# joejep/FOCNeRF

Hardware: AMD Instinct MI355X
Metric: train_samples_per_sec (higher is better)
Workload: dtype f16

## Files before the change

focnerf_amd/_lib.py:

```python
import ctypes
import os

import torch

_HERE = os.path.dirname(os.path.abspath(__file__))
LIB_PATH = os.environ.get("FOCNERF_LIB_PATH") or os.path.join(_HERE, "libfocnerf_hip.so")

c_u8p = ctypes.c_void_p
c_vp = ctypes.c_void_p
u32 = ctypes.c_uint32
u64 = ctypes.c_uint64
f32 = ctypes.c_float
i32 = ctypes.c_int

FOC_F32 = 0
FOC_F16 = 1



class FocOccTrainNode(ctypes.Structure):
    _fields_ = [
        ("struct_bytes", u32),
        ("n_rays", u32), ("max_steps", u32), ("cascade", u32), ("grid_size", u32), ("cap", u32), ("pad_align", u32),
        ("bound", f32), ("dt_gamma", f32), ("min_near", f32),
# ... 47 lines not shown
    _fields_ = [
        ("mask", c_vp), ("offsets", c_vp), ("sigma_c", c_vp), ("rgb_c", c_vp),
        ("m_occ", u32), ("density_scale", f32), ("thresh", f32), ("sigma_gain", f32),
    ]


SIGNATURES = {
    "foc_abi_version": (i32, []),
    "foc_last_error": (ctypes.c_char_p, []),
    "foc_arch": (ctypes.c_char_p, []),
    "foc_near_far_from_aabb": (i32, [c_vp, c_vp, c_vp, u32, f32, c_vp, c_vp, c_vp]),
    "foc_sph_from_ray": (i32, [c_vp, c_vp, f32, u32, c_vp, c_vp]),
    "foc_morton3D": (i32, [c_vp, u32, c_vp, c_vp]),
    "foc_morton3D_invert": (i32, [c_vp, u32, c_vp, c_vp]),
    "foc_packbits": (i32, [c_vp, u32, f32, c_vp, c_vp]),
    "foc_march_rays_train": (i32, [c_vp, c_vp, c_vp, f32, f32, u32, u32, u32, u32, u32, c_vp, c_vp,
                                   c_vp, c_vp, c_vp, c_vp, c_vp, c_vp, c_vp, c_vp]),
    "foc_march_rays_train_field": (i32, [c_vp, c_vp, c_vp, f32, f32, u32, u32, u32, u32, u32, c_vp, c_vp,
                                         c_vp, c_vp, c_vp, c_vp, c_vp, c_vp, c_vp, u32, c_vp, f32, c_vp]),
    "foc_set_option": (i32, [ctypes.c_char_p, i32]),
    "foc_get_option": (i32, [ctypes.c_char_p, c_vp]),
    "foc_guard_pick_device": (i32, [i32, i32, i32, i32]),
    "foc_grid_forward_index_path": (i32, [u32, u32, u32]),
    "foc_view_tile_order": (i32, [c_vp, u32, u32, u32, c_vp, c_vp, c_vp]),
    "foc_occ_train_forward": (i32, [ctypes.POINTER(FocOccTrainNode), c_vp]),
    "foc_occ_train_backward": (i32, [ctypes.POINTER(FocOccTrainNode), c_vp]),
    "foc_occ_train_forward_pad31": (i32, [ctypes.POINTER(FocOccTrainNode), f32, c_vp]),
    "foc_occ_train_backward_pad31": (i32, [ctypes.POINTER(FocOccTrainNode), f32, c_vp]),
    "foc_occ_train_forward_obj": (i32, [ctypes.POINTER(FocOccTrainNode), ctypes.POINTER(FocOccTrainObject), c_vp]),
    "foc_occ_train_backward_obj": (i32, [ctypes.POINTER(FocOccTrainNode), ctypes.POINTER(FocOccTrainObject), c_vp]),
    "foc_occ_tail_forward_sumsq": (i32, [c_vp, c_vp, u32, c_vp, c_vp, u32, u32, f32, f32, c_vp, f32, c_vp, c_vp, c_vp, c_vp, c_vp, c_vp, c_vp, c_vp]),
    "foc_occ_tail_backward_sumsq": (i32, [c_vp, c_vp, c_vp, c_vp, u32, c_vp, c_vp, c_vp, c_vp, c_vp, u32, u32, f32, f32, c_vp, f32, c_vp, c_vp, c_vp, c_vp]),
    "foc_occ_tail_forward": (i32, [c_vp, c_vp, u32, c_vp, c_vp, u32, u32, f32, f32, c_vp, f32, c_vp, c_vp, c_vp, c_vp, c_vp, c_vp, c_vp]),
    "foc_occ_tail_backward": (i32, [c_vp, c_vp, c_vp, c_vp, u32, c_vp, c_vp, c_vp, c_vp, c_vp, u32, u32, f32, f32, c_vp, f32, c_vp, c_vp, c_vp]),
    "foc_occ_tail_forward_dist": (i32, [c_vp, c_vp, u32, c_vp, c_vp, u32, u32, f32, f32, c_vp, f32, c_vp, c_vp, c_vp, c_vp, c_vp, c_vp, c_vp, c_vp, c_vp,
                                        c_vp]),
    "foc_occ_tail_backward_dist": (i32, [c_vp, c_vp, c_vp, c_vp, u32, c_vp, c_vp, c_vp, c_vp, c_vp, u32, u32, f32, f32, c_vp, f32, c_vp, c_vp, c_vp, c_vp,
                                         c_vp, c_vp, c_vp]),
    "foc_occ_tail_forward_depth": (i32, [c_vp, c_vp, u32, c_vp, c_vp, u32, u32, f32, f32, c_vp, f32, c_vp, c_vp, c_vp, c_vp, c_vp, c_vp, c_vp, c_vp, c_vp,
                                         c_vp, c_vp]),
    "foc_occ_tail_backward_depth": (i32, [c_vp, c_vp, c_vp, c_vp, u32, c_vp, c_vp, c_vp, c_vp, c_vp, u32, u32, f32, f32, c_vp, f32, c_vp, c_vp, c_vp, c_vp,
                                          c_vp, c_vp, c_vp, c_vp, c_vp, c_vp, c_vp]),
    "foc_occ_train_forward_tail": (i32, [ctypes.POINTER(FocOccTrainNode), ctypes.POINTER(FocOccTrainObject), f32, ctypes.POINTER(FocOccTrainTail), c_vp]),
    "foc_occ_train_backward_tail": (i32, [ctypes.POINTER(FocOccTrainNode), ctypes.POINTER(FocOccTrainObject), f32, ctypes.POINTER(FocOccTrainTail), c_vp]),
    "foc_march_rays_train_scratch_bytes": (u64, [u32, u32]),
    "foc_composite_rays_train_forward": (i32, [c_vp, c_vp, c_vp, c_vp, u32, u32, f32, c_vp, c_vp, c_vp, c_vp]),
# ... 223 lines not shown
```

focnerf_amd/csrc/combine.hip:

```cpp
#include "common.h"
#include "fs_common.h"
#include <string.h>
#include <cmath>

static thread_local char g_err[512] = "";

void foc_set_error(const char *fmt, ...) {
    va_list ap;
    va_start(ap, fmt);
    vsnprintf(g_err, sizeof(g_err), fmt, ap);
    va_end(ap);
}

__global__ void __launch_bounds__(256) k_combine_select(const float *__restrict__ dens, const float *__restrict__ rgb,
                                                        float *__restrict__ max_dens, float *__restrict__ best_rgb, uint64_t n) {
    for (uint64_t i = (uint64_t)blockIdx.x * 256 + threadIdx.x; i < n; i += (uint64_t)gridDim.x * 256) {
        const float d = dens[i], m = max_dens[i];
        if (d > m) { best_rgb[i * 3] = rgb[i * 3]; best_rgb[i * 3 + 1] = rgb[i * 3 + 1]; best_rgb[i * 3 + 2] = rgb[i * 3 + 2]; }
        max_dens[i] = (d != d || m != m) ? __builtin_nanf("") : (d > m ? d : m);
    }
}

__global__ void __launch_bounds__(256) k_combine_pack(const float *__restrict__ dens, uint32_t rank, uint64_t *__restrict__ keys, uint64_t n) {
    for (uint64_t i = (uint64_t)blockIdx.x * 256 + threadIdx.x; i < n; i += (uint64_t)gridDim.x * 256) {
// ... 338 lines not shown
    bool take = false;
    if (s0 + lane < n) {
        const T a_raw = sig_new[s0 + lane];
        const float a = (float)a_raw, b = (float)sig_best[s0 + lane];
        take = (a != a) || (b == b && a >= b);
        if (take) sig_best[s0 + lane] = a_raw;
    }
    const uint64_t rows = __ballot(take);
    const uint32_t live = (uint32_t)(n - s0 < 64u ? n - s0 : 64u);
    const uint64_t base = s0 * width;
    for (uint32_t e = lane; e < live * width; e += 64u)
        if ((rows >> (e / width)) & 1ull) feat_best[base + e] = feat_new[base + e];
}

#include <stdlib.h>
#include <string.h>
#include <atomic>
#include <mutex>
struct FocOptionRow { const char *name; std::atomic<int> value; };
static FocOptionRow foc_option_table[FOC_OPT_COUNT] = {
    {"FOC_MLP_BWD_FUSED", 1}, {"FOC_FIELD_FWD_FUSED", 1}, {"FOC_GB_MERGE_MAX_RES", 480}, {"FOC_GB_FACTORED", 1}, {"FOC_GB_TAIL_SPLIT", 16}, {"FOC_GRID_FUSE_SMALL", 1},
    {"FOC_GRID_PAIRS", 1}, {"FOC_GRID_FAST", 1}, {"FOC_MARCH_SERIAL", -1}, {"FOC_MARCH_RAYS_ROW_MAX", 131072}, {"FOC_OCC_MARCH_FORM", -1},
    {"FOC_OCC_SAMPLE_MAJOR", 1}, {"FOC_OCC_FIELD_PIECE", 1 << 23}, {"FOC_DETERMINISTIC", 0},
};
static int foc_option_parse(int which, const char *text) {
    if (which == FOC_OPT_OCC_MARCH_FORM) {
        if (text[0] == 't') return 0;
        if (text[0] == 'r') return 1;
        if (text[0] == 'l') return 2;
        if (text[0] == 's') return 3;
    }
    return atoi(text);
}
static void foc_options_init() {
    static std::once_flag once;
    std::call_once(once, [] {
        for (int i = 0; i < FOC_OPT_COUNT; i++) {
            const char *e = getenv(foc_option_table[i].name);
            if (e && e[0]) foc_option_table[i].value.store(foc_option_parse(i, e), std::memory_order_relaxed);
        }
    });
}
int foc_opt(FocOpt which) { foc_options_init(); return foc_option_table[which].value.load(std::memory_order_relaxed); }

extern "C" {

// ... 223 lines not shown
```

focnerf_amd/csrc/common.h:

```cpp
#pragma once
#include <hip/hip_runtime.h>
#include <hip/hip_fp16.h>
#include <stdint.h>
#include <stdio.h>
#include <stdarg.h>
#include "../../include/focnerf.h"

#define FOC_WAVE 64

void foc_set_error(const char *fmt, ...);

enum FocOpt {
    FOC_OPT_MLP_BWD_FUSED,
    FOC_OPT_FIELD_FWD_FUSED,
    FOC_OPT_GB_MERGE_MAX_RES,
    FOC_OPT_GB_FACTORED,
    FOC_OPT_GB_TAIL_SPLIT,
    FOC_OPT_GRID_FUSE_SMALL,
    FOC_OPT_GRID_PAIRS,
    FOC_OPT_GRID_FAST,
    FOC_OPT_MARCH_SERIAL,
    FOC_OPT_MARCH_RAYS_ROW_MAX,
    FOC_OPT_OCC_MARCH_FORM,
    FOC_OPT_OCC_SAMPLE_MAJOR,
    FOC_OPT_OCC_FIELD_PIECE,
    FOC_OPT_DETERMINISTIC,
    FOC_OPT_COUNT
};
int foc_opt(FocOpt which);

#define FOC_REQUIRE(cond, code, ...)                    \
    do {                                                \
        if (!(cond)) {                                  \
            foc_set_error(__VA_ARGS__);                 \
            return (code);                              \
        }                                               \
    } while (0)

#define FOC_CHECK_LAUNCH(name)                                                     \
    do {                                                                           \
        hipError_t e_ = hipGetLastError();                                         \
        if (e_ != hipSuccess) {                                                    \
            foc_set_error("%s: launch failed: %s", name, hipGetErrorString(e_));   \
            return FOC_E_LAUNCH;                                                   \
        }                                                                          \
    } while (0)

static inline int foc_guard_pick(bool stream_is_null, int stream_device, int pointer_device, int current_device) {
    if (!stream_is_null && stream_device >= 0) return stream_device;
// ... 93 lines not shown
```

focnerf_amd/csrc/ge_common.h:

```cpp
#pragma once
#include "common.h"
#include <math.h>
#include <stdlib.h>

#define GE_MAX_LEVELS 32

struct GeLevels {
    float scale[GE_MAX_LEVELS];
    uint32_t resolution[GE_MAX_LEVELS];
    uint32_t merge_max_res;
};

__device__ __forceinline__ float ge_opaque(float v) { asm volatile("" : "+v"(v)); return v; }

template <typename T> struct GeT;
template <> struct GeT<float> {
    static __device__ __forceinline__ float ld(const float *p) { return *p; }
    static __device__ __forceinline__ void st(float *p, float v) { *p = v; }
};
template <> struct GeT<__half> {
    static __device__ __forceinline__ float ld(const __half *p) { return __half2float(*p); }
    static __device__ __forceinline__ void st(__half *p, float v) { *p = __float2half_rn(ge_opaque(v)); }
};

// ... 287 lines not shown
            pgl[gd] = pos_grid[gd] + 1;
            const uint32_t rr = ge_index(dim, gridtype, align_corners, hashmap_size, resolution, pgl);
            float vl[C], vr[C];
            GeVec<T, C>::ld(table + (uint64_t)rl * C, vl);
            GeVec<T, C>::ld(table + (uint64_t)rr * C, vr);
#pragma unroll
            for (uint32_t c = 0; c < C; c++) rg[c] = fmaf(w * (vr[c] - vl[c]), pos_deriv[gd], rg[c]);
        }
#pragma unroll
        for (uint32_t c = 0; c < C; c++) GeT<T>::st(dy + gd * C + c, rg[c]);
    }
}

__host__ __device__ __forceinline__ bool ge_level_hashed(uint32_t hashmap_size, uint32_t resolution, uint32_t &st1, uint32_t &st2) {
    const uint32_t r1 = resolution + 1u;
    uint32_t stride = 1u;
    st1 = st2 = 0u;
    if (stride <= hashmap_size) stride *= r1;
    if (stride <= hashmap_size) { st1 = stride; stride *= r1; }
    if (stride <= hashmap_size) { st2 = stride; stride *= r1; }
    return stride > hashmap_size;
}

__device__ __forceinline__ void ge_forward_hash3(const float (&x)[3], bool oob, const uint32_t *__restrict__ tw, uint32_t hashmap_size, bool hashed,
                                                 uint32_t st1, uint32_t st2, float scale, __half *__restrict__ out) {
    if (oob) { *reinterpret_cast<uint32_t *>(out) = 0u; return; }
    float pos[3];
    uint32_t pg[3];
#pragma unroll
    for (int d = 0; d < 3; d++) {
        const float p = fmaf(x[d], scale, 0.5f);
        pg[d] = (uint32_t)p;
        pos[d] = __builtin_amdgcn_fractf(p);
    }
    const char *tb = reinterpret_cast<const char *>(tw);
    uint32_t b0[4];
    uint2 wide[4];
    uint32_t nar[4] = {0u, 0u, 0u, 0u};
    bool pr[4];
    if (hashmap_size <= (1u << 22)) {
        const uint32_t x4 = pg[0] << 2;
        uint32_t yz4[4];
        if (hashed) {
            const uint32_t m = hashmap_size - 1u, m4 = m << 2;
            const uint32_t p1 = (2654435761u & m) << 2, p2 = (805459861u & m) << 2;
            const uint32_t t1 = __umul24(pg[1], p1), t2 = __umul24(pg[2], p2);
            yz4[0] = t1 ^ t2; yz4[1] = (t1 + p1) ^ t2; yz4[2] = t1 ^ (t2 + p2); yz4[3] = (t1 + p1) ^ (t2 + p2);
#pragma unroll
            for (int j = 0; j < 4; j++) b0[j] = (x4 ^ yz4[j]) & m4;
#pragma unroll
            for (int j = 0; j < 4; j++) wide[j] = *reinterpret_cast<const uint2 *>(tb + (b0[j] & ~7u));
            const bool even = (x4 & 4u) == 0u;
            if (!even) {
#pragma unroll
                for (int j = 0; j < 4; j++) nar[j] = *reinterpret_cast<const uint32_t *>(tb + (((x4 + 4u) ^ yz4[j]) & m4));
            }
#pragma unroll
            for (int j = 0; j < 4; j++) pr[j] = even;
        } else {
            const uint32_t s1 = st1 << 2, s2 = st2 << 2;
            const uint32_t t1 = __umul24(pg[1], s1), t2 = __umul24(pg[2], s2);
            yz4[0] = t1 + t2; yz4[1] = (t1 + s1) + t2; yz4[2] = t1 + (t2 + s2); yz4[3] = (t1 + s1) + (t2 + s2);
// ... 15 lines not shown
        for (int j = 0; j < 4; j++) b0[j] = ((pg[0] ^ yz[j]) & mask) << 2;
#pragma unroll
        for (int j = 0; j < 4; j++) wide[j] = *reinterpret_cast<const uint2 *>(tb + (b0[j] & ~7u));
        const bool even = (pg[0] & 1u) == 0u;
        if (!even) {
#pragma unroll
            for (int j = 0; j < 4; j++) nar[j] = *reinterpret_cast<const uint32_t *>(tb + ((((pg[0] + 1u) ^ yz[j]) & mask) << 2));
        }
#pragma unroll
        for (int j = 0; j < 4; j++) pr[j] = even;
    } else {
        const uint32_t t1 = pg[1] * st1, t2 = pg[2] * st2;
        const uint32_t yz[4] = {t1 + t2, (t1 + st1) + t2, t1 + (t2 + st2), (t1 + st1) + (t2 + st2)};
#pragma unroll
        for (int j = 0; j < 4; j++) b0[j] = (pg[0] + yz[j]) << 2;
#pragma unroll
        for (int j = 0; j < 4; j++) wide[j] = *reinterpret_cast<const uint2 *>(tb + (b0[j] & ~7u));
#pragma unroll
        for (int j = 0; j < 4; j++) {
            pr[j] = (b0[j] & 4u) == 0u;
            if (!pr[j]) nar[j] = *reinterpret_cast<const uint32_t *>(tb + (b0[j] + 4u));
        }
    }
    const float wx[2] = {1 - pos[0], pos[0]}, wy[2] = {1 - pos[1], pos[1]}, wz[2] = {1 - pos[2], pos[2]};
    float res0 = 0.0f, res1 = 0.0f;
#pragma unroll
    for (int j = 0; j < 4; j++) {
        const bool odd = (b0[j] & 4u) != 0u;
        const uint32_t v0 = odd ? wide[j].y : wide[j].x;
        const uint32_t v1 = pr[j] ? (odd ? wide[j].x : wide[j].y) : nar[j];
        const __half2 h0 = *reinterpret_cast<const __half2 *>(&v0), h1 = *reinterpret_cast<const __half2 *>(&v1);
        const float w0 = (wx[0] * wy[j & 1]) * wz[j >> 1], w1 = (wx[1] * wy[j & 1]) * wz[j >> 1];
        res0 = fmaf(w0, __low2float(h0), res0); res1 = fmaf(w0, __high2float(h0), res1);
        res0 = fmaf(w1, __low2float(h1), res0); res1 = fmaf(w1, __high2float(h1), res1);
    }
    *reinterpret_cast<__half2 *>(out) = __halves2half2(__float2half_rn(ge_opaque(res0)), __float2half_rn(ge_opaque(res1)));
}

__host__ __device__ __forceinline__ bool ge_hash3_admits(uint32_t hashmap_size, bool hashed) {
    return (!hashed || (hashmap_size & (hashmap_size - 1u)) == 0u) && hashmap_size <= (1u << 30);
}

template <typename T, typename DIM, uint32_t C>
__device__ __forceinline__ void ge_forward_level(DIM dim, const float (&x)[DIM::MAX], bool oob, const T *__restrict__ grid, uint32_t off0, uint32_t hashmap_size,
                                                 float scale, uint32_t resolution, T *__restrict__ out, T *__restrict__ dy, uint32_t gridtype,
                                                 bool align_corners, uint32_t interp, uint32_t pairs) {
    if constexpr (sizeof(T) == 2 && DIM::STATIC == 3 && C == 2) {
        const bool aligned = ((off0 | hashmap_size) & 1u) == 0u;
        if (pairs == 2u && aligned) {
            uint32_t st1, st2;
            const bool hashed = ge_level_hashed(hashmap_size, resolution, st1, st2);
            if (ge_hash3_admits(hashmap_size, hashed)) {
                ge_forward_hash3(x, oob, reinterpret_cast<const uint32_t *>(grid) + off0, hashmap_size, hashed, st1, st2, scale,
                                 reinterpret_cast<__half *>(out));
                return;
            }
        }
        if (pairs && aligned) {
            ge_forward_one<T, DIM, C, true>(dim, x, oob, grid + (uint64_t)off0 * C, hashmap_size, scale, resolution, out, dy, gridtype, align_corners, interp);
            return;
        }
    }
    ge_forward_one<T, DIM, C, false>(dim, x, oob, grid + (uint64_t)off0 * C, hashmap_size, scale, resolution, out, dy, gridtype, align_corners, interp);
}

__device__ __forceinline__ void ge_walk(uint32_t f, uint32_t chunks, uint32_t lc, uint32_t &chunk, uint32_t &l0, uint32_t &l1) {
    const uint32_t grp = f / chunks;
    chunk = f - grp * chunks;
    if (lc < 2u) { l0 = grp; l1 = grp + 1u; }
    else if (grp == 0u) { l0 = 0u; l1 = lc; }
    else { l0 = lc + grp - 1u; l1 = l0 + 1u; }
}

template <typename T, typename DIM, uint32_t C>
__global__ void __launch_bounds__(256) k_grid_fwd_lbc(const float *__restrict__ inputs, const T *__restrict__ grid,
                                                      const int32_t *__restrict__ offsets, T *__restrict__ outputs,
                                                      uint32_t B, uint32_t L, GeLevels lv, T *__restrict__ dy_dx,
                                                      uint32_t gridtype, bool align_corners, uint32_t interp, uint32_t chunks, uint32_t plain,
                                                      uint32_t pairs, uint32_t lc) {
    const DIM dim;
    uint32_t chunk, l0, l1;
    if (plain) ge_walk(blockIdx.x, chunks, lc, chunk, l0, l1);
    else { if (!ge_decode_block(blockIdx.x, chunks, L, l0, chunk)) return; l1 = l0 + 1u; }
    const uint32_t b = chunk * 256 + threadIdx.x;
    if (b >= B || l0 >= L) return;
    float x[DIM::MAX];
    const bool oob = ge_load_point(dim, inputs, b, x);
    for (uint32_t level = l0; level < l1; level++) {
        const uint32_t off0 = (uint32_t)offsets[level];
        const uint32_t hashmap_size = (uint32_t)offsets[level + 1] - off0;
        T *dy = dy_dx ? dy_dx + ((uint64_t)b * L + level) * dim.n() * C : nullptr;
        ge_forward_level<T, DIM, C>(dim, x, oob, grid, off0, hashmap_size, lv.scale[level], lv.resolution[level], outputs + ((uint64_t)level * B + b) * C, dy,
                                    gridtype, align_corners, interp, pairs);
    }
// ... 142 lines not shown
    GeLevels lv;
    uint32_t gridtype, interp;
    bool ac, bl;
    const void *inputs;
    const void *emb;
    const int32_t *offsets;
    void *out;
    const void *grad;
    void *dy_dx, *grad_inputs;
    float weight;
    hipStream_t st;
};

static uint32_t ge_small_levels(uint32_t L, const GeLevels &lv) {
    const int on = foc_opt(FOC_OPT_GRID_FUSE_SMALL);
    if (!on) return 0u;
    const uint32_t finest = on > 1 ? (uint32_t)on : 160u;
    const uint32_t most = L / 2;
    uint32_t lc = 0;
    while (lc < most && lc < L && lv.resolution[lc] <= finest) lc++;
    return lc >= 2u ? lc : 0u;
}

static bool ge_pairs_enabled() {
    return foc_opt(FOC_OPT_GRID_PAIRS) != 0;
}
static uint32_t ge_pairs_mode(const void *emb, const void *dy_dx, size_t elem, uint32_t D, uint32_t C, uint32_t gridtype, bool ac, uint32_t interp) {
    const int fast = foc_opt(FOC_OPT_GRID_FAST);
    if (!ge_pairs_enabled() || ((uintptr_t)emb & 7u) != 0u || dy_dx) return 0u;
    return (fast && elem == 2 && D == 3 && C == 2 && gridtype == 0u && !ac && interp == 0u) ? 2u : 1u;
}

template <typename T, typename DIM, uint32_t C>
static int ge_forward_launch(const GeCall &a) {
    if constexpr (DIM::STATIC == 0) {
        hipLaunchKernelGGL((k_grid_fwd_pl<T, C>), dim3(foc_div_up(a.B, 256), a.L), dim3(256), 0, a.st, (const float *)a.inputs, (const T *)a.emb, a.offsets, (T *)a.out,
                           a.B, a.L, a.lv, (T *)a.dy_dx, a.gridtype, a.ac, a.interp, a.bl, a.D);
    } else if (a.bl) {
        const uint64_t total = (uint64_t)a.B * a.L;
        const uint32_t grid = (uint32_t)((total + 255) / 256 > 0x7FFFFFFFull ? 0x7FFFFFFFull : (total + 255) / 256);
        hipLaunchKernelGGL((k_grid_fwd_bl<T, DIM, C>), dim3(grid), dim3(256), 0, a.st, (const float *)a.inputs, (const T *)a.emb, a.offsets, (T *)a.out, a.B, a.L, a.lv,
                           (T *)a.dy_dx, a.gridtype, a.ac, a.interp);
    } else {
        const int lm_plain = 1;
        const uint32_t chunks = foc_div_up(a.B, 256);
        const uint32_t lc = lm_plain ? ge_small_levels(a.L, a.lv) : 0u;
// ... 61 lines not shown
```

focnerf_amd/csrc/gridencoder.hip:

```cpp
#include "common.h"
#include <math.h>
#include <stdlib.h>

#include "ge_common.h"

#define GB_SEG_SHIFT 13u
#define GB_SEG (1u << GB_SEG_SHIFT)
#define GB_MAX_SEGS 64u
#define GB_CHUNK 32768u

struct GbHeader {
    uint32_t counts[GE_MAX_LEVELS * GB_MAX_SEGS];
    uint32_t base[GE_MAX_LEVELS * GB_MAX_SEGS + 1];
    uint32_t cursor[GE_MAX_LEVELS * GB_MAX_SEGS];
    uint32_t chunk_prefix[GE_MAX_LEVELS * GB_MAX_SEGS + 1];
};

struct GbSizes { uint32_t size[GE_MAX_LEVELS]; };

template <typename T> struct GbRec;
template <> struct GbRec<__half> { static constexpr uint32_t bytes = 8; };
template <> struct GbRec<float> { static constexpr uint32_t bytes = 12; };

__device__ __forceinline__ void gb_weighted_grads(const uint32_t (&pg)[3], const float (&pf)[3], float g0, float g1, float (&pv)[16]) {
// ... 156 lines not shown
                        const uint32_t s0 = rows[2 * j] >> GB_SEG_SHIFT, s1 = rows[2 * j + 1] >> GB_SEG_SHIFT;
                        atomicAdd(&hist[level * GB_MAX_SEGS + s0], 1u);
                        if (s0 != s1) atomicAdd(&hist[level * GB_MAX_SEGS + s1], 1u);
                    }
                }
            }
        }
    }
    __syncthreads();
    for (uint32_t i = slot_lo + threadIdx.x; i < slot_hi; i += THREADS) {
        const uint32_t hcount = hist[i];
        if (hcount) (void)__hip_atomic_fetch_add(&hdr->counts[i], hcount, __ATOMIC_RELAXED, __HIP_MEMORY_SCOPE_AGENT);
        wg_hist[(uint64_t)i * n_wg + tile] = hcount;
    }
}

__global__ void __launch_bounds__(GB_PMS_WG) k_gbin_count_pt(const float *__restrict__ inputs, const int32_t *__restrict__ offsets, GbHeader *__restrict__ hdr,
                                                             uint32_t *__restrict__ wg_hist, uint32_t B, uint32_t L, GeLevels lv, uint32_t gridtype,
                                                             bool align_corners, uint32_t interp) {
    __shared__ uint32_t hist[GE_MAX_LEVELS * GB_MAX_SEGS];
    gb_count_tile<GB_PMS_WG>(hist, blockIdx.x, gridDim.x, inputs, offsets, hdr, wg_hist, B, L, lv, gridtype, align_corners, interp, 0u, L);
}

template <typename T>
__global__ void __launch_bounds__(256) k_grid_fwd_counted(const float *__restrict__ inputs, const T *__restrict__ grid, const int32_t *__restrict__ offsets,
                                                          T *__restrict__ outputs, uint32_t B, uint32_t L, GeLevels lv, uint32_t gridtype, bool align_corners,
                                                          uint32_t interp, uint32_t chunks, uint32_t pairs, GbHeader *__restrict__ hdr,
                                                          uint32_t *__restrict__ wg_hist, uint32_t n_tiles, uint32_t period, uint32_t w0, uint32_t lc, uint32_t csplit) {
    __shared__ uint32_t hist[GE_MAX_LEVELS * GB_MAX_SEGS];
    const uint32_t n_count = n_tiles * csplit;
    uint32_t f = blockIdx.x;
    if (blockIdx.x >= w0) {
        const uint32_t g = blockIdx.x - w0, q = g / period, r = g - q * period;
        if (r == period - 1u && q < n_count) {
            const uint32_t part = q % csplit;
            gb_count_tile<256>(hist, q / csplit, n_tiles, inputs, offsets, hdr, wg_hist, B, L, lv, gridtype, align_corners, interp, (part * L) / csplit, ((part + 1u) * L) / csplit);
            return;
        }
        f = blockIdx.x - min(q, n_count);
    }
    uint32_t chunk, l0, l1;
    ge_walk(f, chunks, lc, chunk, l0, l1);
    const uint32_t b = chunk * 256 + threadIdx.x;
    if (l0 >= L || b >= B) return;
    float x[3];
    const bool oob = ge_load_point(GeDimCT<3>(), inputs, b, x);
    for (uint32_t level = l0; level < l1; level++) {
        const uint32_t off0 = (uint32_t)offsets[level];
        const uint32_t hashmap_size = (uint32_t)offsets[level + 1] - off0;
        ge_forward_level<T, GeDimCT<3>, 2>(GeDimCT<3>(), x, oob, grid, off0, hashmap_size, lv.scale[level], lv.resolution[level], outputs + ((uint64_t)level * B + b) * 2,
                                  (T *)nullptr, gridtype, align_corners, interp, pairs);
    }
}

template <typename T>
__global__ void __launch_bounds__(GB_PMS_WG, (sizeof(T) == 2 ? 8 : 4)) k_gbin_scatter_pms(
    const T *__restrict__ grad, const float *__restrict__ inputs, const int32_t *__restrict__ offsets, const GbHeader *__restrict__ hdr,
    const uint32_t *__restrict__ wg_base, void *__restrict__ recs, uint64_t max_recs, uint32_t B, uint32_t L, GeLevels lv, uint32_t gridtype,
    bool align_corners, uint32_t interp, bool grad_bl, uint32_t fact_mask, GbSizes sz, uint32_t n_tiles, uint32_t n_whole, uint32_t split) {
    uint32_t tile = blockIdx.x, l_begin = 0u, l_end = L;
    if (blockIdx.x >= n_whole) {
        const uint32_t r = blockIdx.x - n_whole, part = r % split;
        tile = n_whole + r / split;
        l_begin = (part * L) / split; l_end = ((part + 1u) * L) / split;
// ... 523 lines not shown
    const uint64_t wg = (uint64_t)foc_div_up(B, GB_PM_TILE) * L * GB_MAX_SEGS * 4;
    if (det) return gb_base_workspace_bytes(B, L, dtype) + gb_det_images(B, L, det) * (GB_SEG * 2 * 8 + GB_SEG / 8);
    return hdr + gb_rec_array_bytes(m, dtype) + 256 + wg + 256;
}
static uint64_t gb_recs_bytes(uint32_t B, uint32_t L, int dtype) {
    const uint64_t m = gb_max_recs(B, L);
    return (gb_rec_array_bytes(m, dtype) + 255) & ~(uint64_t)255;
}

static int gb_count(const float *inputs, const int32_t *offsets, uint32_t B, uint32_t L, const GeLevels &lv, uint32_t gridtype, bool ac, uint32_t interp,
                    int dtype, void *workspace, hipStream_t st) {
    GbHeader *hdr = reinterpret_cast<GbHeader *>(workspace);
    void *recs = reinterpret_cast<char *>(workspace) + ((sizeof(GbHeader) + 255) & ~(uint64_t)255);
    if (foc_zero_async(hdr->counts, sizeof(hdr->counts), st) != hipSuccess) { foc_set_error("grid_encode_backward: memset failed"); return FOC_E_LAUNCH; }
    const uint32_t n_wg = foc_div_up(B, GB_PM_TILE);
    uint32_t *wg_hist = reinterpret_cast<uint32_t *>(reinterpret_cast<char *>(recs) + gb_recs_bytes(B, L, dtype));
    hipLaunchKernelGGL(k_gbin_count_pt, dim3(n_wg), dim3(GB_PMS_WG), 0, st, inputs, offsets, hdr, wg_hist, B, L, lv, gridtype, ac, interp);
    FOC_CHECK_LAUNCH("grid_encode_backward(count)");
    hipLaunchKernelGGL(k_gbin_scans, dim3(L * GB_MAX_SEGS + 1), dim3(256), 0, st, hdr, wg_hist, n_wg, L);
    FOC_CHECK_LAUNCH("grid_encode_backward(scans)");
    return FOC_OK;
}

template <typename T>
static int gb_forward_counted(const float *inputs, const void *emb, const int32_t *offsets, void *outputs, uint32_t B, uint32_t L, const GeLevels &lv,
                              uint32_t gridtype, bool ac, uint32_t interp, void *workspace, hipStream_t st) {
    GbHeader *hdr = reinterpret_cast<GbHeader *>(workspace);
    void *recs = reinterpret_cast<char *>(workspace) + ((sizeof(GbHeader) + 255) & ~(uint64_t)255);
    if (foc_zero_async(hdr->counts, sizeof(hdr->counts), st) != hipSuccess) { foc_set_error("grid_encode_forward_counted: memset failed"); return FOC_E_LAUNCH; }
    const uint32_t n_tiles = foc_div_up(B, GB_PM_TILE), chunks = foc_div_up(B, 256);
    const uint32_t lc = ge_small_levels(L, lv);
    const uint32_t groups = lc >= 2u ? L - lc + 1u : L;
    const uint32_t fwd_blocks = chunks * groups;
    const uint32_t lo = groups >= 4 ? groups / 2 : 0, hi = groups >= 4 ? groups - 1 : groups;
    const uint32_t csplit = L >= 4u ? 4u : 1u, n_count = n_tiles * csplit;
    const uint32_t w0 = lo * chunks, fit = ((hi - lo) * chunks) / n_count + 1u, period = (fit & 1u) ? fit : fit - 1u;
    uint32_t *wg_hist = reinterpret_cast<uint32_t *>(reinterpret_cast<char *>(recs) + gb_recs_bytes(B, L, sizeof(T) == 2 ? FOC_F16 : FOC_F32));
    hipLaunchKernelGGL((k_grid_fwd_counted<T>), dim3(fwd_blocks + n_count), dim3(256), 0, st, inputs, (const T *)emb, offsets, (T *)outputs, B, L, lv, gridtype, ac,
                       interp, chunks, sizeof(T) == 2 ? ge_pairs_mode(emb, nullptr, sizeof(T), 3, 2, gridtype, ac, interp) : 0u, hdr, wg_hist, n_tiles, period, w0, lc, csplit);
    FOC_CHECK_LAUNCH("grid_encode_forward_counted");
    hipLaunchKernelGGL(k_gbin_scans, dim3(L * GB_MAX_SEGS + 1), dim3(256), 0, st, hdr, wg_hist, n_tiles, L);
    FOC_CHECK_LAUNCH("grid_encode_forward_counted(scans)");
    return FOC_OK;
}

static uint32_t gb_fact_mask(uint32_t L, const GeLevels &lv, const int32_t *offsets_host, uint32_t gridtype, bool ac, int dtype) {
    const int on = foc_opt(FOC_OPT_GB_FACTORED);
    if (!on || dtype != FOC_F16 || gridtype != 0u) return 0u;
    uint32_t m = 0;
    for (uint32_t l = 0; l < L && l < 32u; l++) {
        const uint32_t size = (uint32_t)(offsets_host[l + 1] - offsets_host[l]);
        const uint32_t r1 = ac ? lv.resolution[l] : lv.resolution[l] + 1u;
        uint32_t stride = 1u;
        for (int d = 0; d < 3; d++) if (stride <= size) stride *= r1;
        const bool hashed = stride > size;
        if (hashed && (size & (size - 1u)) == 0u && size >= GB_SEG && lv.resolution[l] > lv.merge_max_res) m |= 1u << l;
    }
    return m;
}

static uint32_t gb_scatter_resident(size_t elem) {
    static uint32_t cus[16];
// ... 61 lines not shown
                            uint32_t C, uint32_t L, float S, uint32_t H, void *dy_dx, uint32_t gridtype, int align_corners,
                            uint32_t interp, int dtype, const int32_t *offsets_host, void *stream) {
    FocDeviceGuard foc_guard_(stream, inputs);
    (void)offsets_host;
    return ge_forward(inputs, embeddings, offsets, outputs, B, D, C, L, S, H, dy_dx, gridtype, align_corners, interp, dtype, false, stream);
}

int foc_grid_encode_forward_bl(const float *inputs, const void *embeddings, const int32_t *offsets, void *outputs, uint32_t B, uint32_t D,
                               uint32_t C, uint32_t L, float S, uint32_t H, void *dy_dx, uint32_t gridtype, int align_corners,
                               uint32_t interp, int dtype, const int32_t *offsets_host, void *stream) {
    FocDeviceGuard foc_guard_(stream, inputs);
    (void)offsets_host;
    return ge_forward(inputs, embeddings, offsets, outputs, B, D, C, L, S, H, dy_dx, gridtype, align_corners, interp, dtype, true, stream);
}

int foc_grid_forward_index_path(uint32_t level_rows, uint32_t resolution, uint32_t level_offset_rows) {
    if (((level_offset_rows | level_rows) & 1u) != 0u) return 0;
    uint32_t st1, st2;
    const bool hashed = ge_level_hashed(level_rows, resolution, st1, st2);
    if (!ge_hash3_admits(level_rows, hashed)) return 0;
    return level_rows <= (1u << 22) ? 2 : 1;
}

int foc_grid_planes_to_rows(const void *planes, void *rows, uint32_t B, uint32_t L, uint32_t unit_bytes, void *stream) {
    FocDeviceGuard foc_guard_(stream, planes);
    if (B == 0) return FOC_OK;
    FOC_REQUIRE(planes && rows, FOC_E_INVALID, "grid_planes_to_rows: null pointer");
    FOC_REQUIRE(L >= 1 && L <= GE_MAX_LEVELS && (unit_bytes == 4 || unit_bytes == 8), FOC_E_INVALID, "grid_planes_to_rows: L in [1,%d], 4- or 8-byte units", GE_MAX_LEVELS);
    hipStream_t st = (hipStream_t)stream;
    if (unit_bytes == 4) hipLaunchKernelGGL((k_planes_to_rows<uint32_t>), dim3(foc_grid_1d(B, 256)), dim3(256), 0, st, (const uint32_t *)planes, (uint32_t *)rows, B, L);
    else hipLaunchKernelGGL((k_planes_to_rows<uint2>), dim3(foc_grid_1d(B, 256)), dim3(256), 0, st, (const uint2 *)planes, (uint2 *)rows, B, L);
    FOC_CHECK_LAUNCH("grid_planes_to_rows");
    return FOC_OK;
}

int foc_grid_rows_to_planes(const void *rows, void *planes, uint32_t B, uint32_t L, uint32_t unit_bytes, void *stream) {
    FocDeviceGuard foc_guard_(stream, rows);
    if (B == 0) return FOC_OK;
    FOC_REQUIRE(planes && rows, FOC_E_INVALID, "grid_rows_to_planes: null pointer");
    FOC_REQUIRE(L >= 1 && L <= GE_MAX_LEVELS && (unit_bytes == 4 || unit_bytes == 8), FOC_E_INVALID, "grid_rows_to_planes: L in [1,%d], 4- or 8-byte units", GE_MAX_LEVELS);
    hipStream_t st = (hipStream_t)stream;
    if (unit_bytes == 4) hipLaunchKernelGGL((k_rows_to_planes<uint32_t>), dim3(foc_grid_1d(B, 256)), dim3(256), 0, st, (const uint32_t *)rows, (uint32_t *)planes, B, L);
    else hipLaunchKernelGGL((k_rows_to_planes<uint2>), dim3(foc_grid_1d(B, 256)), dim3(256), 0, st, (const uint2 *)rows, (uint2 *)planes, B, L);
    FOC_CHECK_LAUNCH("grid_rows_to_planes");
    return FOC_OK;
}
// ... 48 lines not shown
                                   uint32_t gridtype, int align_corners, uint32_t interp, int dtype, const int32_t *offsets_host, void *workspace,
                                   uint64_t workspace_bytes, void *stream) {
    FocDeviceGuard foc_guard_(stream, inputs);
    if (B == 0) return FOC_OK;
    FOC_REQUIRE(inputs && offsets && workspace && offsets_host, FOC_E_INVALID, "grid_encode_backward_count: null pointer");
    const int rc = gb_check(B, D, C, L, S, H, gridtype, interp, dtype, offsets_host, workspace_bytes);
    if (rc) return rc;
    GeLevels lv;
    ge_make_levels(L, S, H, lv);
    return gb_count(inputs, offsets, B, L, lv, gridtype, align_corners != 0, interp, dtype, workspace, (hipStream_t)stream);
}

int foc_grid_encode_forward_counted(const float *inputs, const void *embeddings, const int32_t *offsets, void *outputs, uint32_t B, uint32_t D, uint32_t C,
                                    uint32_t L, float S, uint32_t H, uint32_t gridtype, int align_corners, uint32_t interp, int dtype,
                                    const int32_t *offsets_host, void *workspace, uint64_t workspace_bytes, void *stream) {
    FocDeviceGuard foc_guard_(stream, inputs);
    if (B == 0) return FOC_OK;
    FOC_REQUIRE(inputs && embeddings && offsets && outputs && workspace && offsets_host, FOC_E_INVALID, "grid_encode_forward_counted: null pointer");
    const int rc = gb_check(B, D, C, L, S, H, gridtype, interp, dtype, offsets_host, workspace_bytes);
    if (rc) return rc;
    GeLevels lv;
    ge_make_levels(L, S, H, lv);
    hipStream_t st = (hipStream_t)stream;
    if (dtype == FOC_F32) return gb_forward_counted<float>(inputs, embeddings, offsets, outputs, B, L, lv, gridtype, align_corners != 0, interp, workspace, st);
    return gb_forward_counted<__half>(inputs, embeddings, offsets, outputs, B, L, lv, gridtype, align_corners != 0, interp, workspace, st);
}

static int gb_entry(const void *grad, const float *inputs, const int32_t *offsets, void *grad_embeddings,
                    uint32_t B, uint32_t D, uint32_t C, uint32_t L, float S, uint32_t H, const void *dy_dx, void *grad_inputs,
                    uint32_t gridtype, int align_corners, uint32_t interp, int dtype, int grad_is_bl,
                    const int32_t *offsets_host, void *workspace, uint64_t workspace_bytes, bool counted, void *stream) {
    if (B == 0) return FOC_OK;
    FOC_REQUIRE(grad && inputs && offsets && grad_embeddings && workspace && offsets_host, FOC_E_INVALID, "grid_encode_backward_binned: null pointer");
    const int det_on = foc_opt(FOC_OPT_DETERMINISTIC);
    FOC_REQUIRE(!(det_on && dtype == FOC_F32), FOC_E_INVALID, "grid_encode_backward_binned: FOC_DETERMINISTIC is set and the fp32-table reduce sums in an "
                "order that depends on timing (its LDS sum is a double atomic); deterministic mode serves fp16 tables");
    const int det = dtype == FOC_F16 && det_on ? (det_on == 2 ? 2 : 1) : 0;
    {
        const int rc0 = gb_check(B, D, C, L, S, H, gridtype, interp, dtype, offsets_host, workspace_bytes, det);
        if (rc0) return rc0;
    }
    GeLevels lv;
    ge_make_levels(L, S, H, lv);
    hipStream_t st = (hipStream_t)stream;
    const bool ac = align_corners != 0, bl = grad_is_bl != 0;
    const uint32_t fact_mask = gb_fact_mask(L, lv, offsets_host, gridtype, ac, dtype);
    GbSizes sz;
    for (uint32_t l = 0; l < GE_MAX_LEVELS; l++) sz.size[l] = l < L ? (uint32_t)(offsets_host[l + 1] - offsets_host[l]) : 0u;
// ... 47 lines not shown
```

include/focnerf.h:

```cpp
#ifndef FOCNERF_H
#define FOCNERF_H

#include <stdint.h>

#ifdef __cplusplus
extern "C" {
#endif

#define FOC_OK            0
#define FOC_E_INVALID     1
#define FOC_E_DTYPE       2
#define FOC_E_LAUNCH      3

#define FOC_F32 0
#define FOC_F16 1

#define FOC_ABI_VERSION 2
int         foc_abi_version(void);
const char *foc_last_error(void);
int foc_set_option(const char *name, int value);
int foc_get_option(const char *name, int *value);
int foc_guard_pick_device(int stream_is_null, int stream_device, int pointer_device, int current_device);
const char *foc_arch(void);

// ... 81 lines not shown
                            float *samples, void *planes, float *sigma, float *rgb,
                            const void *embeddings, const int32_t *offsets, const int32_t *offsets_host, uint32_t L, float S, uint32_t base_res,
                            const void *sigma_weights, uint32_t sigma_layers, const void *color_weights, uint32_t color_layers, uint32_t activation,
                            const void *obj_feat, float T_thresh, float *weights_sum, float *depth, float *image, void *scratch, uint32_t flags,
                            int32_t *deaths, uint32_t deaths_base, uint32_t deaths_len, float input_pad, void *stream);

int foc_compact_alive(const int32_t *rays_alive, uint32_t n_alive, int32_t *out, int32_t *n_out,
                      int32_t *scratch, void *stream);


int foc_grid_encode_forward(const float *inputs, const void *embeddings, const int32_t *offsets,
                            void *outputs, uint32_t B, uint32_t D, uint32_t C, uint32_t L,
                            float S, uint32_t H, void *dy_dx, uint32_t gridtype,
                            int align_corners, uint32_t interp, int dtype,
                            const int32_t *offsets_host, void *stream);

int foc_grid_encode_forward_bl(const float *inputs, const void *embeddings, const int32_t *offsets,
                               void *outputs, uint32_t B, uint32_t D, uint32_t C, uint32_t L,
                               float S, uint32_t H, void *dy_dx, uint32_t gridtype,
                               int align_corners, uint32_t interp, int dtype,
                               const int32_t *offsets_host, void *stream);
int foc_grid_planes_to_rows(const void *planes, void *rows, uint32_t B, uint32_t L, uint32_t unit_bytes, void *stream);
int foc_grid_forward_index_path(uint32_t level_rows, uint32_t resolution, uint32_t level_offset_rows);
int foc_grid_rows_to_planes(const void *rows, void *planes, uint32_t B, uint32_t L, uint32_t unit_bytes, void *stream);

int foc_grid_encode_backward(const void *grad, const float *inputs, const void *embeddings,
                             const int32_t *offsets, void *grad_embeddings,
                             uint32_t B, uint32_t D, uint32_t C, uint32_t L, float S, uint32_t H,
                             const void *dy_dx, void *grad_inputs, uint32_t gridtype,
                             int align_corners, uint32_t interp, int dtype, int grad_is_bl,
                             const int32_t *offsets_host, void *stream);

uint64_t foc_grid_encode_backward_workspace_bytes(uint32_t B, uint32_t D, uint32_t C, uint32_t L, int dtype);
int foc_grid_encode_backward_binned(const void *grad, const float *inputs, const void *embeddings,
                                    const int32_t *offsets, void *grad_embeddings,
                                    uint32_t B, uint32_t D, uint32_t C, uint32_t L, float S, uint32_t H,
                                    const void *dy_dx, void *grad_inputs, uint32_t gridtype,
                                    int align_corners, uint32_t interp, int dtype, int grad_is_bl,
                                    const int32_t *offsets_host, void *workspace, uint64_t workspace_bytes,
                                    void *stream);

int foc_grid_encode_forward_counted(const float *inputs, const void *embeddings, const int32_t *offsets, void *outputs,
                                    uint32_t B, uint32_t D, uint32_t C, uint32_t L, float S, uint32_t H,
                                    uint32_t gridtype, int align_corners, uint32_t interp, int dtype,
                                    const int32_t *offsets_host, void *workspace, uint64_t workspace_bytes, void *stream);
int foc_grid_encode_backward_count(const float *inputs, const int32_t *offsets, uint32_t B, uint32_t D, uint32_t C,
// ... 346 lines not shown
```

Baseline: 1.397 billion.

## Let small grid levels ride on large-level blocks in counted forward

Adds a ride plan that hands the small (dense) levels to the work groups that process hashed large levels. Each host group issues its large-level gathers first, computes the rider small levels while those loads are in flight, then finishes the large level. This cuts the number of launched groups and hides gather latency. It adds the planning logic, a RIDE kernel variant and an option (default 5), and it depends on the fp16 pairs path and on hash3 admissibility for every level.

```diff
diff --git a/focnerf_amd/_lib.py b/focnerf_amd/_lib.py
--- a/focnerf_amd/_lib.py
+++ b/focnerf_amd/_lib.py
@@ -93,6 +93,7 @@
     "foc_get_option": (i32, [ctypes.c_char_p, c_vp]),
     "foc_guard_pick_device": (i32, [i32, i32, i32, i32]),
     "foc_grid_forward_index_path": (i32, [u32, u32, u32]),
+    "foc_grid_forward_counted_walk": (i32, [u32, f32, u32, u32, i32, u32, i32, c_vp, c_vp, c_vp]),
     "foc_view_tile_order": (i32, [c_vp, u32, u32, u32, c_vp, c_vp, c_vp]),
     "foc_occ_train_forward": (i32, [ctypes.POINTER(FocOccTrainNode), c_vp]),
     "foc_occ_train_backward": (i32, [ctypes.POINTER(FocOccTrainNode), c_vp]),
diff --git a/focnerf_amd/csrc/combine.hip b/focnerf_amd/csrc/combine.hip
--- a/focnerf_amd/csrc/combine.hip
+++ b/focnerf_amd/csrc/combine.hip
@@ -384,6 +384,7 @@
     {"FOC_MLP_BWD_FUSED", 1}, {"FOC_FIELD_FWD_FUSED", 1}, {"FOC_GB_MERGE_MAX_RES", 480}, {"FOC_GB_FACTORED", 1}, {"FOC_GB_TAIL_SPLIT", 16}, {"FOC_GRID_FUSE_SMALL", 1},
     {"FOC_GRID_PAIRS", 1}, {"FOC_GRID_FAST", 1}, {"FOC_MARCH_SERIAL", -1}, {"FOC_MARCH_RAYS_ROW_MAX", 131072}, {"FOC_OCC_MARCH_FORM", -1},
     {"FOC_OCC_SAMPLE_MAJOR", 1}, {"FOC_OCC_FIELD_PIECE", 1 << 23}, {"FOC_DETERMINISTIC", 0},
+    {"FOC_GRID_RIDE_SMALL", 5},
 };
 static int foc_option_parse(int which, const char *text) {
     if (which == FOC_OPT_OCC_MARCH_FORM) {
diff --git a/focnerf_amd/csrc/common.h b/focnerf_amd/csrc/common.h
--- a/focnerf_amd/csrc/common.h
+++ b/focnerf_amd/csrc/common.h
@@ -25,6 +25,7 @@
     FOC_OPT_OCC_SAMPLE_MAJOR,
     FOC_OPT_OCC_FIELD_PIECE,
     FOC_OPT_DETERMINISTIC,
+    FOC_OPT_GRID_RIDE_SMALL,
     FOC_OPT_COUNT
 };
 int foc_opt(FocOpt which);
diff --git a/focnerf_amd/csrc/ge_common.h b/focnerf_amd/csrc/ge_common.h
--- a/focnerf_amd/csrc/ge_common.h
+++ b/focnerf_amd/csrc/ge_common.h
@@ -1,5 +1,6 @@
 #pragma once
 #include "common.h"
+#include "ge_walk.h"
 #include <math.h>
 #include <stdlib.h>
 
@@ -333,10 +334,15 @@
     return stride > hashmap_size;
 }
 
-__device__ __forceinline__ void ge_forward_hash3(const float (&x)[3], bool oob, const uint32_t *__restrict__ tw, uint32_t hashmap_size, bool hashed,
-                                                 uint32_t st1, uint32_t st2, float scale, __half *__restrict__ out) {
-    if (oob) { *reinterpret_cast<uint32_t *>(out) = 0u; return; }
+struct GeHash3 {
     float pos[3];
+    uint32_t b0[4];
+    uint2 wide[4];
+    uint32_t nar[4];
+    bool pr[4];
+};
+__device__ __forceinline__ void ge_hash3_issue(const float (&x)[3], const uint32_t *__restrict__ tw, uint32_t hashmap_size, bool hashed, uint32_t st1, uint32_t st2,
+                                               float scale, float (&pos)[3], uint32_t (&b0)[4], uint2 (&wide)[4], uint32_t (&nar)[4], bool (&pr)[4]) {
     uint32_t pg[3];
 #pragma unroll
     for (int d = 0; d < 3; d++) {
@@ -345,10 +351,6 @@
         pos[d] = __builtin_amdgcn_fractf(p);
     }
     const char *tb = reinterpret_cast<const char *>(tw);
-    uint32_t b0[4];
-    uint2 wide[4];
-    uint32_t nar[4] = {0u, 0u, 0u, 0u};
-    bool pr[4];
     if (hashmap_size <= (1u << 22)) {
         const uint32_t x4 = pg[0] << 2;
         uint32_t yz4[4];
@@ -410,6 +412,9 @@
             if (!pr[j]) nar[j] = *reinterpret_cast<const uint32_t *>(tb + (b0[j] + 4u));
         }
     }
+}
+__device__ __forceinline__ void ge_hash3_finish(const float (&pos)[3], const uint32_t (&b0)[4], const uint2 (&wide)[4], const uint32_t (&nar)[4], const bool (&pr)[4],
+                                                __half *__restrict__ out) {
     const float wx[2] = {1 - pos[0], pos[0]}, wy[2] = {1 - pos[1], pos[1]}, wz[2] = {1 - pos[2], pos[2]};
     float res0 = 0.0f, res1 = 0.0f;
 #pragma unroll
@@ -424,9 +429,30 @@
     }
     *reinterpret_cast<__half2 *>(out) = __halves2half2(__float2half_rn(ge_opaque(res0)), __float2half_rn(ge_opaque(res1)));
 }
+__device__ __forceinline__ void ge_forward_hash3(const float (&x)[3], bool oob, const uint32_t *__restrict__ tw, uint32_t hashmap_size, bool hashed,
+                                                 uint32_t st1, uint32_t st2, float scale, __half *__restrict__ out) {
+    if (oob) { *reinterpret_cast<uint32_t *>(out) = 0u; return; }
+    float pos[3];
+    uint32_t b0[4];
+    uint2 wide[4];
+    uint32_t nar[4] = {0u, 0u, 0u, 0u};
+    bool pr[4];
+    ge_hash3_issue(x, tw, hashmap_size, hashed, st1, st2, scale, pos, b0, wide, nar, pr);
+    ge_hash3_finish(pos, b0, wide, nar, pr, out);
+}
 
 __host__ __device__ __forceinline__ bool ge_hash3_admits(uint32_t hashmap_size, bool hashed) {
     return (!hashed || (hashmap_size & (hashmap_size - 1u)) == 0u) && hashmap_size <= (1u << 30);
+}
+
+static inline bool ge_hash3_serves_all(const int32_t *offsets_host, uint32_t L, const GeLevels &lv) {
+    for (uint32_t l = 0; l < L; l++) {
+        const uint32_t off0 = (uint32_t)offsets_host[l], hashmap_size = (uint32_t)offsets_host[l + 1] - off0;
+        uint32_t st1, st2;
+        const bool hashed = ge_level_hashed(hashmap_size, lv.resolution[l], st1, st2);
+        if (((off0 | hashmap_size) & 1u) != 0u || !ge_hash3_admits(hashmap_size, hashed)) return false;
+    }
+    return true;
 }
 
 template <typename T, typename DIM, uint32_t C>
@@ -450,14 +476,6 @@
         }
     }
     ge_forward_one<T, DIM, C, false>(dim, x, oob, grid + (uint64_t)off0 * C, hashmap_size, scale, resolution, out, dy, gridtype, align_corners, interp);
-}
-
-__device__ __forceinline__ void ge_walk(uint32_t f, uint32_t chunks, uint32_t lc, uint32_t &chunk, uint32_t &l0, uint32_t &l1) {
-    const uint32_t grp = f / chunks;
-    chunk = f - grp * chunks;
-    if (lc < 2u) { l0 = grp; l1 = grp + 1u; }
-    else if (grp == 0u) { l0 = 0u; l1 = lc; }
-    else { l0 = lc + grp - 1u; l1 = l0 + 1u; }
 }
 
 template <typename T, typename DIM, uint32_t C>
@@ -646,6 +664,12 @@
     return lc >= 2u ? lc : 0u;
 }
 
+static GeRide ge_ride(const int32_t *offsets_host, uint32_t L, const GeLevels &lv, uint32_t lc) {
+    uint32_t n_dense = 0, st1, st2;
+    while (n_dense < lc && !ge_level_hashed((uint32_t)offsets_host[n_dense + 1] - (uint32_t)offsets_host[n_dense], lv.resolution[n_dense], st1, st2)) n_dense++;
+    return ge_ride_plan(foc_opt(FOC_OPT_GRID_RIDE_SMALL), L, lc, n_dense);
+}
+
 static bool ge_pairs_enabled() {
     return foc_opt(FOC_OPT_GRID_PAIRS) != 0;
 }
diff --git a/focnerf_amd/csrc/ge_walk.h b/focnerf_amd/csrc/ge_walk.h
--- /dev/null
+++ b/focnerf_amd/csrc/ge_walk.h
@@ -0,0 +1,76 @@
+#pragma once
+#include <stdint.h>
+
+#if defined(__HIPCC__)
+#define GE_HD __host__ __device__ __forceinline__
+#else
+#define GE_HD static inline
+#endif
+
+GE_HD void ge_walk(uint32_t f, uint32_t chunks, uint32_t lc, uint32_t &chunk, uint32_t &l0, uint32_t &l1) {
+    const uint32_t grp = f / chunks;
+    chunk = f - grp * chunks;
+    if (lc < 2u) { l0 = grp; l1 = grp + 1u; }
+    else if (grp == 0u) { l0 = 0u; l1 = lc; }
+    else { l0 = lc + grp - 1u; l1 = l0 + 1u; }
+}
+
+struct GeRide {
+    uint32_t nr;
+    uint32_t hosts;
+};
+GE_HD uint32_t ge_popc(uint32_t v) { uint32_t n = 0; for (; v; v &= v - 1u) n++; return n; }
+GE_HD uint32_t ge_ride_groups(uint32_t L, uint32_t lc, GeRide rd) { return (L - lc) + (rd.nr < lc ? 1u : 0u); }
+GE_HD void ge_walk_paired(uint32_t f, uint32_t chunks, uint32_t lc, GeRide rd, uint32_t &chunk, uint32_t &l0, uint32_t &l1, uint32_t &r0, uint32_t &r1) {
+    const uint32_t grp = f / chunks, shared = rd.nr < lc ? 1u : 0u;
+    chunk = f - grp * chunks;
+    r0 = r1 = 0u;
+    if (shared && grp == 0u) { l0 = rd.nr; l1 = lc; return; }
+    const uint32_t p = grp - shared;
+    l0 = lc + p; l1 = l0 + 1u;
+    if (p < 32u && ((rd.hosts >> p) & 1u)) {
+        const uint32_t n = ge_popc(rd.hosts), j = ge_popc(rd.hosts & ((1u << p) - 1u));
+        r0 = (j * rd.nr) / n; r1 = ((j + 1u) * rd.nr) / n;
+    }
+}
+
+struct GeCountPlan { uint32_t n_count, csplit, w0, period, lo, hi; };
+GE_HD GeCountPlan ge_count_plan(uint32_t groups, uint32_t chunks, uint32_t n_tiles, uint32_t L) {
+    GeCountPlan c;
+    c.lo = groups >= 4u ? groups / 2u : 0u;
+    c.hi = groups >= 4u ? groups - 1u : groups;
+    c.csplit = L >= 4u ? 4u : 1u;
+    c.n_count = n_tiles * c.csplit;
+    c.w0 = c.lo * chunks;
+    const uint32_t fit = ((c.hi - c.lo) * chunks) / c.n_count + 1u;
+    c.period = (fit & 1u) ? fit : fit - 1u;
+    return c;
+}
+GE_HD bool ge_count_slot(uint32_t g, uint32_t period, uint32_t n_count, uint32_t &q) {
+    q = g / period;
+    return g - q * period == period - 1u && q < n_count;
+}
+
+GE_HD GeRide ge_ride_plan(int mode, uint32_t L, uint32_t lc, uint32_t n_dense) {
+    GeRide rd = {0u, 0u};
+    const int kind = mode & 3;
+    if (mode <= 0 || mode > 15 || kind == 0 || lc < 2u || L <= lc || L - lc > 32u) return rd;
+    const uint32_t nf = L - lc, all = nf >= 32u ? ~0u : (1u << nf) - 1u;
+    rd.nr = kind == 1 ? (n_dense < lc ? n_dense : lc) : lc;
+    if (rd.nr == 0u) return rd;
+    uint32_t cand = kind == 3 ? all & ~((1u << (nf / 2u)) - 1u) : all;
+    if (mode & 4) {
+        const uint32_t shared = rd.nr < lc ? 1u : 0u;
+        const GeCountPlan c = ge_count_plan(nf + shared, 1u, 1u, L);
+        for (uint32_t g = c.lo; g < c.hi; g++) if (g >= shared) cand &= ~(1u << (g - shared));
+    }
+    if (mode & 8) cand &= ~(1u << (nf - 1u));
+    if (cand == 0u) cand = 1u << (nf - 1u);
+    rd.hosts = cand;
+    if (kind == 1) {
+        uint32_t n = 0u;
+        rd.hosts = 0u;
+        for (uint32_t p = 0; p < nf && n < rd.nr; p++) if ((cand >> p) & 1u) { rd.hosts |= 1u << p; n++; }
+    }
+    return rd;
+}
diff --git a/focnerf_amd/csrc/gridencoder.hip b/focnerf_amd/csrc/gridencoder.hip
--- a/focnerf_amd/csrc/gridencoder.hip
+++ b/focnerf_amd/csrc/gridencoder.hip
@@ -202,17 +202,18 @@
     gb_count_tile<GB_PMS_WG>(hist, blockIdx.x, gridDim.x, inputs, offsets, hdr, wg_hist, B, L, lv, gridtype, align_corners, interp, 0u, L);
 }
 
-template <typename T>
+template <typename T, bool RIDE = false>
 __global__ void __launch_bounds__(256) k_grid_fwd_counted(const float *__restrict__ inputs, const T *__restrict__ grid, const int32_t *__restrict__ offsets,
                                                           T *__restrict__ outputs, uint32_t B, uint32_t L, GeLevels lv, uint32_t gridtype, bool align_corners,
                                                           uint32_t interp, uint32_t chunks, uint32_t pairs, GbHeader *__restrict__ hdr,
-                                                          uint32_t *__restrict__ wg_hist, uint32_t n_tiles, uint32_t period, uint32_t w0, uint32_t lc, uint32_t csplit) {
+                                                          uint32_t *__restrict__ wg_hist, uint32_t n_tiles, uint32_t period, uint32_t w0, uint32_t lc, uint32_t csplit,
+                                                          GeRide ride) {
     __shared__ uint32_t hist[GE_MAX_LEVELS * GB_MAX_SEGS];
     const uint32_t n_count = n_tiles * csplit;
     uint32_t f = blockIdx.x;
     if (blockIdx.x >= w0) {
-        const uint32_t g = blockIdx.x - w0, q = g / period, r = g - q * period;
-        if (r == period - 1u && q < n_count) {
+        uint32_t q;
+        if (ge_count_slot(blockIdx.x - w0, period, n_count, q)) {
             const uint32_t part = q % csplit;
             gb_count_tile<256>(hist, q / csplit, n_tiles, inputs, offsets, hdr, wg_hist, B, L, lv, gridtype, align_corners, interp, (part * L) / csplit, ((part + 1u) * L) / csplit);
             return;
@@ -220,6 +221,35 @@
         f = blockIdx.x - min(q, n_count);
     }
     uint32_t chunk, l0, l1;
+    if constexpr (RIDE) {
+        uint32_t r0, r1;
+        ge_walk_paired(f, chunks, lc, ride, chunk, l0, l1, r0, r1);
+        const uint32_t b = chunk * 256 + threadIdx.x;
+        if (l0 >= L || b >= B) return;
+        float x[3];
+        const bool oob = ge_load_point(GeDimCT<3>(), inputs, b, x);
+        const uint32_t *tw = reinterpret_cast<const uint32_t *>(grid);
+        __half *planes = reinterpret_cast<__half *>(outputs);
+        GeHash3 g = {};
+        if (r1 > r0 && !oob) {
+            const uint32_t off0 = (uint32_t)offsets[l0], hashmap_size = (uint32_t)offsets[l0 + 1] - off0;
+            uint32_t st1, st2;
+            const bool hashed = ge_level_hashed(hashmap_size, lv.resolution[l0], st1, st2);
+            ge_hash3_issue(x, tw + off0, hashmap_size, hashed, st1, st2, lv.scale[l0], g.pos, g.b0, g.wide, g.nar, g.pr);
+        }
+        for (uint32_t level = r0 < r1 ? r0 : l0; level < (r0 < r1 ? r1 : l1); level++) {
+            const uint32_t off0 = (uint32_t)offsets[level], hashmap_size = (uint32_t)offsets[level + 1] - off0;
+            uint32_t st1, st2;
+            const bool hashed = ge_level_hashed(hashmap_size, lv.resolution[level], st1, st2);
+            ge_forward_hash3(x, oob, tw + off0, hashmap_size, hashed, st1, st2, lv.scale[level], planes + ((uint64_t)level * B + b) * 2);
+        }
+        if (r1 > r0) {
+            __half *out = planes + ((uint64_t)l0 * B + b) * 2;
+            if (oob) *reinterpret_cast<uint32_t *>(out) = 0u;
+            else ge_hash3_finish(g.pos, g.b0, g.wide, g.nar, g.pr, out);
+        }
+        return;
+    }
     ge_walk(f, chunks, lc, chunk, l0, l1);
     const uint32_t b = chunk * 256 + threadIdx.x;
     if (l0 >= L || b >= B) return;
@@ -789,22 +819,29 @@
     return FOC_OK;
 }
 
+static GeRide gb_forward_ride(uint32_t pairs, const int32_t *offsets_host, uint32_t L, const GeLevels &lv, uint32_t lc) {
+    if (pairs != 2u || lc < 2u || !ge_hash3_serves_all(offsets_host, L, lv)) return GeRide{0u, 0u};
+    return ge_ride(offsets_host, L, lv, lc);
+}
+
 template <typename T>
 static int gb_forward_counted(const float *inputs, const void *emb, const int32_t *offsets, void *outputs, uint32_t B, uint32_t L, const GeLevels &lv,
-                              uint32_t gridtype, bool ac, uint32_t interp, void *workspace, hipStream_t st) {
+                              uint32_t gridtype, bool ac, uint32_t interp, const int32_t *offsets_host, void *workspace, hipStream_t st) {
     GbHeader *hdr = reinterpret_cast<GbHeader *>(workspace);
     void *recs = reinterpret_cast<char *>(workspace) + ((sizeof(GbHeader) + 255) & ~(uint64_t)255);
     if (foc_zero_async(hdr->counts, sizeof(hdr->counts), st) != hipSuccess) { foc_set_error("grid_encode_forward_counted: memset failed"); return FOC_E_LAUNCH; }
     const uint32_t n_tiles = foc_div_up(B, GB_PM_TILE), chunks = foc_div_up(B, 256);
     const uint32_t lc = ge_small_levels(L, lv);
-    const uint32_t groups = lc >= 2u ? L - lc + 1u : L;
+    const uint32_t pairs = sizeof(T) == 2 ? ge_pairs_mode(emb, nullptr, sizeof(T), 3, 2, gridtype, ac, interp) : 0u;
+    const GeRide ride = gb_forward_ride(pairs, offsets_host, L, lv, lc);
+    const uint32_t groups = ride.nr ? ge_ride_groups(L, lc, ride) : lc >= 2u ? L - lc + 1u : L;
     const uint32_t fwd_blocks = chunks * groups;
-    const uint32_t lo = groups >= 4 ? groups / 2 : 0, hi = groups >= 4 ? groups - 1 : groups;
-    const uint32_t csplit = L >= 4u ? 4u : 1u, n_count = n_tiles * csplit;
-    const uint32_t w0 = lo * chunks, fit = ((hi - lo) * chunks) / n_count + 1u, period = (fit & 1u) ? fit : fit - 1u;
+    const GeCountPlan cp = ge_count_plan(groups, chunks, n_tiles, L);
     uint32_t *wg_hist = reinterpret_cast<uint32_t *>(reinterpret_cast<char *>(recs) + gb_recs_bytes(B, L, sizeof(T) == 2 ? FOC_F16 : FOC_F32));
-    hipLaunchKernelGGL((k_grid_fwd_counted<T>), dim3(fwd_blocks + n_count), dim3(256), 0, st, inputs, (const T *)emb, offsets, (T *)outputs, B, L, lv, gridtype, ac,
-                       interp, chunks, sizeof(T) == 2 ? ge_pairs_mode(emb, nullptr, sizeof(T), 3, 2, gridtype, ac, interp) : 0u, hdr, wg_hist, n_tiles, period, w0, lc, csplit);
+    auto kernel = k_grid_fwd_counted<T, false>;
+    if constexpr (sizeof(T) == 2) { if (ride.nr) kernel = k_grid_fwd_counted<T, true>; }
+    hipLaunchKernelGGL(kernel, dim3(fwd_blocks + cp.n_count), dim3(256), 0, st, inputs, (const T *)emb, offsets, (T *)outputs, B, L, lv, gridtype, ac, interp, chunks, pairs,
+                       hdr, wg_hist, n_tiles, cp.period, cp.w0, lc, cp.csplit, ride);
     FOC_CHECK_LAUNCH("grid_encode_forward_counted");
     hipLaunchKernelGGL(k_gbin_scans, dim3(L * GB_MAX_SEGS + 1), dim3(256), 0, st, hdr, wg_hist, n_tiles, L);
     FOC_CHECK_LAUNCH("grid_encode_forward_counted(scans)");
@@ -912,6 +949,19 @@
     return level_rows <= (1u << 22) ? 2 : 1;
 }
 
+int foc_grid_forward_counted_walk(uint32_t L, float S, uint32_t H, uint32_t gridtype, int align_corners, uint32_t interp, int dtype, const int32_t *offsets_host,
+                                  uint32_t *riders, uint32_t *hosts) {
+    FOC_REQUIRE(offsets_host && riders && hosts, FOC_E_INVALID, "grid_forward_counted_walk: null pointer");
+    FOC_REQUIRE(L >= 1 && L <= GE_MAX_LEVELS, FOC_E_INVALID, "grid_forward_counted_walk: L in [1,%d]", GE_MAX_LEVELS);
+    GeLevels lv;
+    ge_make_levels(L, S, H, lv);
+    const uint32_t pairs = dtype == FOC_F16 ? ge_pairs_mode(nullptr, nullptr, 2, 3, 2, gridtype, align_corners != 0, interp) : 0u;
+    const GeRide ride = gb_forward_ride(pairs, offsets_host, L, lv, ge_small_levels(L, lv));
+    *riders = ride.nr;
+    *hosts = ride.hosts;
+    return FOC_OK;
+}
+
 int foc_grid_planes_to_rows(const void *planes, void *rows, uint32_t B, uint32_t L, uint32_t unit_bytes, void *stream) {
     FocDeviceGuard foc_guard_(stream, planes);
     if (B == 0) return FOC_OK;
@@ -1006,8 +1056,8 @@
     GeLevels lv;
     ge_make_levels(L, S, H, lv);
     hipStream_t st = (hipStream_t)stream;
-    if (dtype == FOC_F32) return gb_forward_counted<float>(inputs, embeddings, offsets, outputs, B, L, lv, gridtype, align_corners != 0, interp, workspace, st);
-    return gb_forward_counted<__half>(inputs, embeddings, offsets, outputs, B, L, lv, gridtype, align_corners != 0, interp, workspace, st);
+    if (dtype == FOC_F32) return gb_forward_counted<float>(inputs, embeddings, offsets, outputs, B, L, lv, gridtype, align_corners != 0, interp, offsets_host, workspace, st);
+    return gb_forward_counted<__half>(inputs, embeddings, offsets, outputs, B, L, lv, gridtype, align_corners != 0, interp, offsets_host, workspace, st);
 }
 
 static int gb_entry(const void *grad, const float *inputs, const int32_t *offsets, void *grad_embeddings,
diff --git a/include/focnerf.h b/include/focnerf.h
--- a/include/focnerf.h
+++ b/include/focnerf.h
@@ -127,6 +127,8 @@
                                const int32_t *offsets_host, void *stream);
 int foc_grid_planes_to_rows(const void *planes, void *rows, uint32_t B, uint32_t L, uint32_t unit_bytes, void *stream);
 int foc_grid_forward_index_path(uint32_t level_rows, uint32_t resolution, uint32_t level_offset_rows);
+int foc_grid_forward_counted_walk(uint32_t L, float S, uint32_t H, uint32_t gridtype, int align_corners, uint32_t interp, int dtype,
+                                  const int32_t *offsets_host, uint32_t *riders, uint32_t *hosts);
 int foc_grid_rows_to_planes(const void *rows, void *planes, uint32_t B, uint32_t L, uint32_t unit_bytes, void *stream);
 
 int foc_grid_encode_backward(const void *grad, const float *inputs, const void *embeddings,
```

Result: faster. 1.411 billion (median of 6 runs) (+1.0%).
